# KwonGihyun/TweedieMix

Measured on AMD Instinct MI355X. Metric: denoise steps/sec @ SDXL 1024^2 K=3 concepts (fusion phase); images/sec at 1/2/4/8 GPUs, higher is better.
Workload: dtype bf16

## Files before the change

include/tmix.h:

```cpp
#ifndef TMIX_H
#define TMIX_H

#include <stdint.h>

#ifdef __cplusplus
extern "C" {
#endif

#define TMIX_VERSION 100

enum { TMIX_OK = 0, TMIX_EINVAL = -1, TMIX_ESHAPE = -2, TMIX_EARCH = -3, TMIX_EALIGN = -4 };
enum { TMIX_F32 = 0, TMIX_F16 = 1, TMIX_BF16 = 2 };

int tmix_version(void);
const char* tmix_last_error_string(void);
int tmix_check_device(void);
void tmix_env_refresh(void);

int tmix_prof_begin(uint64_t* slots, int capacity, int detail);
int tmix_prof_end(void);

enum { TMIX_STEP_FUSION = 0, TMIX_STEP_PLAIN = 1, TMIX_STEP_RESAMPLE = 2 };
int tmix_fused_tweedie_step(const float* x, const void* eps, int eps_dtype, const float* masks,
                            float* out_x, float* out_x0, int K, int channels, int64_t hw, int mode,
// ... 9 lines not shown
                                     int64_t keep_eps_seed_stride, const float* keep_w, int64_t keep_w_seed_stride, void* stream);
int tmix_fused_tweedie_step_ms_dev(const float* x, const void* eps, int eps_dtype, const float* masks,
                                   int64_t mask_seed_stride, float* out_x, float* out_x0, float* x0_prev, int K, int channels,
                                   int64_t hw, int mode, int rows, int seeds, const float* params, void* stream);
int64_t tmix_cfg_rescale_ws_doubles(int rows, int seeds);
int tmix_cfg_rescale_factors(const void* eps, int eps_dtype, float* factors, double* ws, int K, int channels, int64_t hw, int mode,
                             int rows, int seeds, const float* params, int g_slot, float phi, void* stream);
int tmix_fused_tweedie_step_rs_dev(const float* x, const void* eps, int eps_dtype, const float* masks,
                                   int64_t mask_seed_stride, float* out_x, float* out_x0, int K, int channels,
                                   int64_t hw, int mode, int rows, int seeds, const float* params, const float* factors, void* stream);
int tmix_fused_tweedie_step_ms_rs_dev(const float* x, const void* eps, int eps_dtype, const float* masks,
                                      int64_t mask_seed_stride, float* out_x, float* out_x0, float* x0_prev, int K, int channels,
                                      int64_t hw, int mode, int rows, int seeds, const float* params, const float* factors, void* stream);
int tmix_step_prologue(const float* x, float* latent, float* t_dev, const float* params, int seeds, int rows,
                       int64_t n, void* stream);
#define TMIX_MAX_WINDOWS 8
int tmix_window_consensus(float* x, int groups, int n_win, const int* win_yx, int C, int h, int w, int canvas_h, int canvas_w,
                          const float* weight, void* stream);
#define TMIX_EDT_NONE (1 << 30)
int tmix_mask_edt(const float* mask, int32_t* d_set, int32_t* d_clear, int n, int h, int w, void* stream);
int tmix_soft_masks(const int32_t* d_set, const int32_t* d_clear, float* out, int n_sets, int K, int h, int w, float feather,
                    float dilate, int normalize, void* stream);
#define TMIX_SHAPE_FILL_HOLES 1
#define TMIX_SHAPE_RESOLVE    2
#define TMIX_SHAPE_MAX_PIXELS 16384
int tmix_mask_label(const float* map, float threshold, int invert, int32_t* label, int n, int h, int w, void* stream);
int tmix_attn_shapes(const float* score, float* out, int n_sets, int km1, int h, int w, float threshold, int flags, void* stream);

int tmix_vpred_step(const void* x, const void* v, void* out, int dtype, int64_t n, float g,
                    float sa, float s1, float sa_next, float s1_next, void* stream);
// ... 76 lines not shown
    int32_t batch_bias_images;
    float* col_stats_out;
    const void* S1; const void* S2;
    int32_t S1_channels, S2_channels;
} tmix_conv_desc;
int tmix_conv3x3_nhwc(const tmix_conv_desc* d, void* stream);
int tmix_conv3x3_nhwc_fp8(const tmix_conv_desc* d, const uint8_t* scale_x, const uint8_t* scale_w, void* stream);
int tmix_conv_resolve_tile(const tmix_conv_desc* d, int fp8_operands);

int tmix_conv_in(const float* x_nchw, const float* w_ohwi, const float* bias, void* y_nhwc,
                 int B, int Cin, int H, int W, int Cout, void* stream);
int tmix_conv_in_pre(const float* x_nchw, const float* w_ohwi, const float* bias, void* y_nhwc,
                     int B, int Cin, int H, int W, int Cout, const float* pre_w, const float* pre_b, void* stream);
int tmix_conv_out(const void* x_nhwc, const void* w_ohwi, const float* bias, float* y_nchw,
                  int B, int Cin, int H, int W, int Cout, void* stream);

int tmix_attn_fwd(const void* Q, int64_t ldq, int64_t strideQ, const void* K, int64_t ldk, int64_t strideK,
                  const void* Vt, int64_t ldvt, int64_t strideVt, void* O, int64_t ldo, int64_t strideO,
                  int B, int H, int Sq, int Skv, float scale, void* stream);
int tmix_attn_fwd_f8(const void* Q, int64_t ldq, int64_t strideQ, const void* K, int64_t ldk, int64_t strideK,
                     const void* Vt, int64_t ldvt, int64_t strideVt, void* O8, int64_t ldo8, void* scales, int64_t ldScale,
                     int B, int H, int Sq, int Skv, float scale, void* stream);
int64_t tmix_attn_split_ws_bytes(int B, int H, int Sq, int Skv);
int tmix_attn_fwd_ws(const void* Q, int64_t ldq, int64_t strideQ, const void* K, int64_t ldk, int64_t strideK,
                     const void* Vt, int64_t ldvt, int64_t strideVt, void* O, int64_t ldo, int64_t strideO,
                     int B, int H, int Sq, int Skv, float scale, void* ws, int64_t ws_bytes, void* stream);
int tmix_attn_fwd_f8_ws(const void* Q, int64_t ldq, int64_t strideQ, const void* K, int64_t ldk, int64_t strideK,
                        const void* Vt, int64_t ldvt, int64_t strideVt, void* O8, int64_t ldo8, void* scales, int64_t ldScale,
                        int B, int H, int Sq, int Skv, float scale, void* ws, int64_t ws_bytes, void* stream);

// ... 56 lines not shown
```

tweediemix_amd/csrc/conv_io.hip:

```cpp
#include "common.h"

namespace {

struct PreMap { float w[16]; float b[4]; int on; };

template <int CIN>
__global__ void __launch_bounds__(256) conv_in_kernel(const float* __restrict__ x, const float* __restrict__ w,
                                                      const float* __restrict__ bias, bf16_t* __restrict__ y,
                                                      int B, int H, int W, int Cout, const PreMap pm) {
    extern __shared__ __attribute__((aligned(16))) float s_w[];
    constexpr int KK = 9 * CIN;
    const int tid = threadIdx.x, lane = tid & 63;
    const int q = __builtin_amdgcn_readfirstlane(tid >> 6);
    for (int i = tid; i < Cout * KK / 4; i += 256) ((float4*)s_w)[i] = ((const float4*)w)[i];
    __syncthreads();
    const int64_t npix = (int64_t)B * H * W;
    for (int64_t tile = blockIdx.x; tile * 64 < npix; tile += gridDim.x) {
    int64_t pix = tile * 64 + lane;
    const bool live = pix < npix;
    if (!live) pix = npix - 1;
    const int b = (int)(pix / ((int64_t)H * W)); const int rem = (int)(pix - (int64_t)b * H * W);
    const int oy = rem / W, ox = rem - oy * W;
    float patch[KK];
#pragma unroll
// ... 31 lines not shown
    }
    }
}

template <int CIN>
int launch_conv_in(unsigned nb, int smem, hipStream_t st, const float* x, const float* w, const float* bias, bf16_t* y, int B, int H, int W, int Cout, const PreMap& pm) {
    static int attr_smem = 0;
    if (smem > 64 * 1024 && smem > attr_smem) {
        hipError_t e = hipFuncSetAttribute((const void*)conv_in_kernel<CIN>, hipFuncAttributeMaxDynamicSharedMemorySize, smem);
        if (e != hipSuccess) TMIX_FAIL((int)e, "hipFuncSetAttribute: %s", hipGetErrorString(e));
        attr_smem = smem;
    }
    conv_in_kernel<CIN><<<nb, 256, smem, st>>>(x, w, bias, y, B, H, W, Cout, pm);
    TMIX_LAUNCH_CHECK();
    return TMIX_OK;
}

__global__ void __launch_bounds__(256) conv_out_kernel(const bf16_t* __restrict__ x, const bf16_t* __restrict__ w,
                                                       const float* __restrict__ bias, float* __restrict__ y,
                                                       int B, int H, int W, int Cin, int Cout) {
    const int lane = threadIdx.x & 63, fr = lane & 15, fg = lane >> 4;
    const int64_t npix = (int64_t)B * H * W;
    const int64_t pbase = ((int64_t)blockIdx.x * 4 + (threadIdx.x >> 6)) * 16;
    if (pbase >= npix) return;
    int64_t pix = pbase + fr; if (pix > npix - 1) pix = npix - 1;
    const int b = (int)(pix / ((int64_t)H * W)); const int rem = (int)(pix - (int64_t)b * H * W);
    const int oy = rem / W, ox = rem - oy * W;
    const int co = fr < Cout ? fr : Cout - 1;
    const bf16_t* wrow = w + (int64_t)co * 9 * Cin;
    f32x4 acc = {0.f, 0.f, 0.f, 0.f};
// ... 49 lines not shown
    PreMap pm = {};
    if (pre_w) {
        pm.on = 1;
        for (int i = 0; i < 16; ++i) pm.w[i] = pre_w[i];
        for (int i = 0; i < 4; ++i) pm.b[i] = pre_b ? pre_b[i] : 0.f;
    }
    hipStream_t st = (hipStream_t)stream;
    bf16_t* y = (bf16_t*)y_nhwc;
    switch (Cin) {
        case 8:  return launch_conv_in<8>(nb, smem, st, x_nchw, w_ohwi, bias, y, B, H, W, Cout, pm);
        case 3:  return launch_conv_in<3>(nb, smem, st, x_nchw, w_ohwi, bias, y, B, H, W, Cout, pm);
        default: return launch_conv_in<4>(nb, smem, st, x_nchw, w_ohwi, bias, y, B, H, W, Cout, pm);
    }
}

extern "C" int tmix_conv_out(const void* x_nhwc, const void* w_ohwi, const float* bias, float* y_nchw,
                             int B, int Cin, int H, int W, int Cout, void* stream) {
    if (!x_nhwc || !w_ohwi || !y_nchw) TMIX_FAIL(TMIX_EINVAL, "conv_out: null pointer");
    if (B <= 0 || H <= 0 || W <= 0 || Cout <= 0 || Cout > 16 || (Cin % 32)) TMIX_FAIL(TMIX_ESHAPE, "conv_out: Cin=%d (%%32) Cout=%d (<=16)", Cin, Cout);
    if (!aligned16(x_nhwc) || !aligned16(w_ohwi)) TMIX_FAIL(TMIX_EALIGN, "conv_out: pointers must be 16-byte aligned");
    const int64_t npix = (int64_t)B * H * W;
    const unsigned nb = (unsigned)((npix + 63) / 64);
    conv_out_kernel<<<nb, 256, 0, (hipStream_t)stream>>>((const bf16_t*)x_nhwc, (const bf16_t*)w_ohwi, bias, y_nchw, B, H, W, Cin, Cout);
    TMIX_LAUNCH_CHECK();
    return TMIX_OK;
}
```

tweediemix_amd/csrc/tweedie_step.hip:

```cpp
#include "common.h"

namespace {

template <int DT> struct EpsT;
template <> struct EpsT<TMIX_F32>  { typedef float  T; static __device__ __forceinline__ float ld(const float* p, int64_t i) { return p[i]; } };
template <> struct EpsT<TMIX_F16>  { typedef __half T; static __device__ __forceinline__ float ld(const __half* p, int64_t i) { return __half2float(p[i]); } };
template <> struct EpsT<TMIX_BF16> { typedef bf16_t T; static __device__ __forceinline__ float ld(const bf16_t* p, int64_t i) { return bf2f(p[i]); } };

template <int DT> __device__ __forceinline__ float rnd(float v) {
    if constexpr (DT == TMIX_F16) {
        asm volatile("" : "+v"(v));
        return __half2float(__float2half_rn(v));
    } else return v;
}

template <int DT> __device__ __forceinline__ float cfg(float eu, float ec, float g) {
    const float d = rnd<DT>(ec - eu);
    const float gd = rnd<DT>(g * d);
    return rnd<DT>(eu + gd);
}

struct KeepArgs { const float* x0; const float* eps; const float* w; int64_t x0_stride, eps_stride, w_stride; };
__device__ __forceinline__ KeepArgs keep_args(const KeepArgs& k) { return k; }
struct RescaleArgs { const float* fac; };
// ... 108 lines not shown
    int64_t bx = (n + 255) / 256; if (bx > 2048) bx = 2048;
    const dim3 grid((unsigned)bx, (unsigned)seeds);
    const T* e = (const T*)eps;
    switch (mode) {
    case TMIX_STEP_FUSION:
        tweedie_step_kernel<DT, TMIX_STEP_FUSION, 1><<<grid, 256, 0, st>>>(x, e, masks, out_x, out_x0, K, n, hw, 0.f, 1.f, 0.f, 1.f, 0.f, 0, prm, rows, mss, kp); break;
    case TMIX_STEP_PLAIN:
        tweedie_step_kernel<DT, TMIX_STEP_PLAIN, 1><<<grid, 256, 0, st>>>(x, e, masks, out_x, out_x0, K, n, hw, 0.f, 1.f, 0.f, 1.f, 0.f, 0, prm, rows, mss, kp); break;
    default:
        tweedie_step_kernel<DT, TMIX_STEP_RESAMPLE, 1><<<grid, 256, 0, st>>>(x, e, masks, out_x, out_x0, K, n, hw, 0.f, 1.f, 0.f, 1.f, 0.f, 0, prm, rows, mss, kp); break;
    }
    TMIX_LAUNCH_CHECK();
    return TMIX_OK;
}

__global__ void __launch_bounds__(256)
step_prologue_kernel(const float* __restrict__ x, float* __restrict__ latent, float* __restrict__ t_dev,
                     const float* __restrict__ prm, int rows, int64_t n) {
    const int64_t sd = blockIdx.y;
    const float4* src = (const float4*)(x + sd * n);
    for (int64_t i = (int64_t)blockIdx.x * blockDim.x + threadIdx.x; i < n / 4; i += (int64_t)gridDim.x * blockDim.x) {
        const float4 v = src[i];
        for (int r = 0; r < rows; ++r) ((float4*)(latent + (sd * rows + r) * n))[i] = v;
    }
    if (blockIdx.x == 0 && threadIdx.x < rows) t_dev[sd * rows + threadIdx.x] = prm[0];
}


template <int DT>
__global__ void __launch_bounds__(256)
vpred_step_kernel(const typename EpsT<DT>::T* __restrict__ x, const typename EpsT<DT>::T* __restrict__ v,
                  typename EpsT<DT>::T* __restrict__ out, int64_t n, float g, float sa, float s1, float sa_n, float s1_n) {
    const int64_t stride = (int64_t)gridDim.x * blockDim.x;
    for (int64_t i = (int64_t)blockIdx.x * blockDim.x + threadIdx.x; i < n; i += stride) {
        const float xv = EpsT<DT>::ld(x, i);
        const float vv = cfg<DT>(EpsT<DT>::ld(v, i), EpsT<DT>::ld(v, n + i), g);
        const float eps = rnd<DT>(rnd<DT>(sa * vv) + rnd<DT>(s1 * xv));
        const float x0 = rnd<DT>(rnd<DT>(sa * xv) - rnd<DT>(s1 * vv));
        StT<DT>::st(out, i, rnd<DT>(rnd<DT>(sa_n * x0) + rnd<DT>(s1_n * eps)));
    }
// ... 181 lines not shown
    }
    TMIX_FAIL(TMIX_EINVAL, "tweedie_step_rs_dev: bad eps dtype %d", eps_dtype);
}

extern "C" int tmix_step_prologue(const float* x, float* latent, float* t_dev, const float* params, int seeds, int rows,
                                  int64_t n, void* stream) {
    if (!x || !latent || !t_dev || !params) TMIX_FAIL(TMIX_EINVAL, "step_prologue: null pointer");
    if (seeds < 1 || seeds > 65535 || rows < 1 || rows > 256 || n < 4 || (n & 3)) TMIX_FAIL(TMIX_ESHAPE, "step_prologue: seeds=%d rows=%d n=%lld (n %% 4 == 0)", seeds, rows, (long long)n);
    if (!aligned16(x) || !aligned16(latent)) TMIX_FAIL(TMIX_EALIGN, "step_prologue: x / latent must be 16-byte aligned");
    int64_t bx = (n / 4 + 255) / 256; if (bx > 256) bx = 256;
    step_prologue_kernel<<<dim3((unsigned)bx, (unsigned)seeds), 256, 0, (hipStream_t)stream>>>(x, latent, t_dev, params, rows, n);
    TMIX_LAUNCH_CHECK();
    return TMIX_OK;
}

extern "C" int tmix_video_step_prologue(const float* x, float* x_u, int64_t clip_stride_u, float* t_u, float* x_c, int64_t clip_stride_c,
                                        float* t_c, const float* params, int videos, int channels, int frames, int64_t hw,
                                        int row_channels, void* stream) {
    if (!x || !x_u || !t_u || !x_c || !t_c || !params) TMIX_FAIL(TMIX_EINVAL, "video_step_prologue: null pointer");
    if (videos < 1 || channels < 1 || frames < 1 || hw < 1 || row_channels < channels)
        TMIX_FAIL(TMIX_ESHAPE, "video_step_prologue: videos=%d channels=%d frames=%d hw=%lld row_channels=%d", videos, channels, frames, (long long)hw, row_channels);
    const int64_t clip = (int64_t)frames * row_channels * hw;
    if (clip_stride_u < clip || clip_stride_c < clip)
        TMIX_FAIL(TMIX_ESHAPE, "video_step_prologue: clip strides %lld / %lld < one clip's %lld floats", (long long)clip_stride_u, (long long)clip_stride_c, (long long)clip);
    const int64_t n = (int64_t)videos * channels * frames * hw;
    int64_t blocks = (n + 255) / 256; if (blocks > 4096) blocks = 4096;
    video_prologue_kernel<<<(unsigned)blocks, 256, 0, (hipStream_t)stream>>>(x, x_u, clip_stride_u, t_u, x_c, clip_stride_c, t_c, params,
                                                                             videos, channels, frames, hw, row_channels, n);
    TMIX_LAUNCH_CHECK();
    return TMIX_OK;
// ... 18 lines not shown
```

tweediemix_amd/lib.py:

```python
from __future__ import annotations

import ctypes as C
import os

_HERE = os.path.dirname(os.path.abspath(__file__))
LIB_PATH = os.path.join(_HERE, "lib", "libtmix_hip.so")
LIB_PATH = os.environ.get("TMIX_LIB", LIB_PATH)

OK, EINVAL, ESHAPE, EARCH, EALIGN = 0, -1, -2, -3, -4
F32, F16, BF16 = 0, 1, 2
STEP_FUSION, STEP_PLAIN, STEP_RESAMPLE = 0, 1, 2
EPI_NONE, EPI_GEGLU, EPI_F32OUT, EPI_GELU, EPI_QUICKGELU = 0, 1, 2, 3, 4
CONV_S1, CONV_S2, CONV_UP2, CONV_T3, CONV_S2A, CONV_UP2F = 0, 1, 2, 3, 4, 5
F8_A_BLOCK_SCALES, F8_GEGLU_OUT, F8_COPY_OUT = 1, 2, 4
MAX_WINDOWS = 8
EDT_NONE = 1 << 30
SHAPE_FILL_HOLES, SHAPE_RESOLVE, SHAPE_MAX_PIXELS = 1, 2, 16384
TILE_AUTO, TILE_COUNT = 0, 26
TILE_CANDIDATES = (1, 2, 3, 4, 5, 7, 12, 13, 14, 15, 16, 17, 18, 19, 20, 21, 22)
TILE_EXCLUSIVE = (13, 14, 15, 22, 24)
TILE_CONV_HALO = 26

i32, i64, f32, vp = C.c_int32, C.c_int64, C.c_float, C.c_void_p

# ... 32 lines not shown
    "tmix_fused_tweedie_step": (C.c_int, [vp, vp, C.c_int, vp, vp, vp, C.c_int, C.c_int, i64, C.c_int,
                                          f32, f32, f32, f32, f32, C.c_int, vp]),
    "tmix_fused_tweedie_step_dev": (C.c_int, [vp, vp, C.c_int, vp, i64, vp, vp, C.c_int, C.c_int, i64, C.c_int, C.c_int,
                                              C.c_int, vp, vp]),
    "tmix_fused_tweedie_step_keep_dev": (C.c_int, [vp, vp, C.c_int, vp, i64, vp, vp, C.c_int, C.c_int, i64, C.c_int, C.c_int,
                                                   C.c_int, vp, vp, i64, vp, i64, vp, i64, vp]),
    "tmix_fused_tweedie_step_ms_dev": (C.c_int, [vp, vp, C.c_int, vp, i64, vp, vp, vp, C.c_int, C.c_int, i64, C.c_int, C.c_int,
                                                 C.c_int, vp, vp]),
    "tmix_cfg_rescale_ws_doubles": (i64, [C.c_int, C.c_int]),
    "tmix_cfg_rescale_factors": (C.c_int, [vp, C.c_int, vp, vp, C.c_int, C.c_int, i64, C.c_int, C.c_int, C.c_int, vp, C.c_int, f32, vp]),
    "tmix_fused_tweedie_step_rs_dev": (C.c_int, [vp, vp, C.c_int, vp, i64, vp, vp, C.c_int, C.c_int, i64, C.c_int, C.c_int,
                                                 C.c_int, vp, vp, vp]),
    "tmix_fused_tweedie_step_ms_rs_dev": (C.c_int, [vp, vp, C.c_int, vp, i64, vp, vp, vp, C.c_int, C.c_int, i64, C.c_int, C.c_int,
                                                    C.c_int, vp, vp, vp]),
    "tmix_step_prologue": (C.c_int, [vp, vp, vp, vp, C.c_int, C.c_int, i64, vp]),
    "tmix_window_consensus": (C.c_int, [vp, C.c_int, C.c_int, C.POINTER(C.c_int32), C.c_int, C.c_int, C.c_int, C.c_int, C.c_int, vp, vp]),
    "tmix_mask_edt": (C.c_int, [vp, vp, vp, C.c_int, C.c_int, C.c_int, vp]),
    "tmix_soft_masks": (C.c_int, [vp, vp, vp, C.c_int, C.c_int, C.c_int, C.c_int, f32, f32, C.c_int, vp]),
    "tmix_mask_label": (C.c_int, [vp, f32, C.c_int, vp, C.c_int, C.c_int, C.c_int, vp]),
    "tmix_attn_shapes": (C.c_int, [vp, vp, C.c_int, C.c_int, C.c_int, C.c_int, f32, C.c_int, vp]),
    "tmix_gemm_bf16": (C.c_int, [C.POINTER(GemmDesc), vp]),
    "tmix_gemm_prefetch_next": (C.c_int, [vp, i64, vp]),
    "tmix_gemm_fp8": (C.c_int, [C.POINTER(GemmDesc), vp, vp, vp]),
    "tmix_gemm_q_cross_attn": (C.c_int, [C.POINTER(GemmDesc), vp, i64, i64, vp, i64, i64, vp, i64, C.c_int, C.c_int, f32, vp]),
    "tmix_quantize_fp8_rows": (C.c_int, [vp, i64, vp, i64, vp, i64, C.c_int, vp]),
    "tmix_conv3x3_nhwc": (C.c_int, [C.POINTER(ConvDesc), vp]),
    "tmix_conv3x3_nhwc_fp8": (C.c_int, [C.POINTER(ConvDesc), vp, vp, vp]),
    "tmix_conv_in": (C.c_int, [vp, vp, vp, vp, C.c_int, C.c_int, C.c_int, C.c_int, C.c_int, vp]),
    "tmix_conv_in_pre": (C.c_int, [vp, vp, vp, vp, C.c_int, C.c_int, C.c_int, C.c_int, C.c_int, vp, vp, vp]),
    "tmix_softmax_rows": (C.c_int, [vp, i64, vp, i64, i64, C.c_int, f32, vp]),
    "tmix_softmax_rows_causal": (C.c_int, [vp, i64, vp, i64, i64, C.c_int, f32, C.c_int, vp]),
    "tmix_softmax_rows_masked": (C.c_int, [vp, i64, vp, i64, i64, C.c_int, C.c_int, f32, vp]),
    "tmix_affine_clamp": (C.c_int, [vp, vp, i64, f32, f32, f32, f32, vp]),
    "tmix_conv_out": (C.c_int, [vp, vp, vp, vp, C.c_int, C.c_int, C.c_int, C.c_int, C.c_int, vp]),
    "tmix_attn_fwd": (C.c_int, [vp, i64, i64, vp, i64, i64, vp, i64, i64, vp, i64, i64,
                                C.c_int, C.c_int, C.c_int, C.c_int, f32, vp]),
    "tmix_attn_fwd_f8": (C.c_int, [vp, i64, i64, vp, i64, i64, vp, i64, i64, vp, i64, vp, i64,
                                   C.c_int, C.c_int, C.c_int, C.c_int, f32, vp]),
    "tmix_attn_split_ws_bytes": (i64, [C.c_int, C.c_int, C.c_int, C.c_int]),
    "tmix_attn_fwd_ws": (C.c_int, [vp, i64, i64, vp, i64, i64, vp, i64, i64, vp, i64, i64,
                                   C.c_int, C.c_int, C.c_int, C.c_int, f32, vp, i64, vp]),
    "tmix_attn_fwd_f8_ws": (C.c_int, [vp, i64, i64, vp, i64, i64, vp, i64, i64, vp, i64, vp, i64,
                                      C.c_int, C.c_int, C.c_int, C.c_int, f32, vp, i64, vp]),
    "tmix_groupnorm_nhwc_launches": (C.c_int, [i64, C.c_int, C.c_int]),
    "tmix_groupnorm_ws_chunks": (C.c_int, [i64]),
    "tmix_groupnorm_ws_floats": (i64, [C.c_int, C.c_int, C.c_int]),
    "tmix_groupnorm_nhwc": (C.c_int, [vp, C.c_int, vp, C.c_int, vp, vp, vp, vp, C.c_int, i64, C.c_int, f32,
                                      C.c_int, vp]),
    "tmix_groupnorm_nhwc_pre": (C.c_int, [vp, C.c_int, vp, C.c_int, vp, vp, vp, vp, C.c_int, i64, C.c_int, f32,
# ... 65 lines not shown
```

tweediemix_amd/ops.py:

```python
from __future__ import annotations

import ctypes as C
import os

import numpy as np
import torch

from . import lib as L

BF16 = torch.bfloat16


def _stream() -> int:
    return torch.cuda.current_stream().cuda_stream


def _p(t):
    return None if t is None else t.data_ptr()


def _need_cuda(*ts):
    for t in ts:
        if t is not None and not t.is_cuda:
            raise L.TmixError("tweediemix_amd ops need device tensors (no CPU fallback exists)")
# ... 477 lines not shown
    return out


def conv_in(x_nchw, w_ohwi, bias, out=None):
    _need_cuda(x_nchw, w_ohwi)
    lib = L.load()
    B, Cin, H, W = x_nchw.shape
    Cout = w_ohwi.shape[0]
    assert x_nchw.dtype == torch.float32 and w_ohwi.dtype == torch.float32 and x_nchw.is_contiguous() and w_ohwi.is_contiguous()
    if out is None:
        out = torch.empty(B, H, W, Cout, device=x_nchw.device, dtype=BF16)
    L.check(lib.tmix_conv_in(_p(x_nchw), _p(w_ohwi), _p(bias), _p(out), B, Cin, H, W, Cout, _stream()), "tmix_conv_in")
    return out


def conv_out(x_nhwc, w_ohwi, bias, out=None):
    _need_cuda(x_nhwc, w_ohwi)
    lib = L.load()
    B, H, W, Cin = x_nhwc.shape
    Cout = w_ohwi.shape[0]
    assert x_nhwc.dtype == BF16 and w_ohwi.dtype == BF16 and x_nhwc.is_contiguous() and w_ohwi.is_contiguous()
    if out is None:
        out = torch.empty(B, Cout, H, W, device=x_nhwc.device, dtype=torch.float32)
    L.check(lib.tmix_conv_out(_p(x_nhwc), _p(w_ohwi), _p(bias), _p(out), B, Cin, H, W, Cout, _stream()), "tmix_conv_out")
    return out


def attention_split_ws(B, H, Sq, Skv, device):
    n = L.load().tmix_attn_split_ws_bytes(B, H, Sq, Skv)
    return torch.zeros(n, device=device, dtype=torch.uint8) if n > 0 else None


def attention(q, k, vt, H, Skv, scale, out=None, f8_out=None, ws=None):
    _need_cuda(q, k, vt)
    lib = L.load()
    B, Sq = q.shape[0], q.shape[1]
    assert q.dtype == BF16 and k.dtype == BF16 and vt.dtype == BF16
    assert q.stride(2) == 1 and k.stride(2) == 1 and vt.stride(2) == 1
    wsa = (ws.data_ptr(), ws.numel()) if ws is not None else (None, 0)
# ... 348 lines not shown
```

tweediemix_amd/sampler.py:

```python
from __future__ import annotations

from types import SimpleNamespace

import torch

from . import lib as L
from . import ops
from .schedule import Schedule
from .guidance import validate_phi
from .solver import SOLVERS, multistep_coeffs
from .unet import KVCache, PlanGroup, TokenMapSpec, TokenPropSpec, UNetPlan, UNetWeights

F32 = torch.float32


def seed_everything(seed: int):
    import random

    import numpy as np
    torch.manual_seed(seed)
    if torch.cuda.is_available():
        torch.cuda.manual_seed(seed)
    random.seed(seed)
    np.random.seed(seed)
# ... 75 lines not shown
                                 + (f"; unknown keys {sorted(extra)}" if extra else ""))
            self.mask_soften = dict(feather=f, dilate=r, normalize=bool(ms.get("normalize", False)))
        self._mask_buf = None
        self.scheduler = Schedule(config.n_timesteps, spacing=timestep_spacing)
        self.skip = self.scheduler.skip
        self.final_alpha_cumprod = self.scheduler.final_alpha_cumprod
        self.h, self.w = config.resolution_h // 8, config.resolution_w // 8
        self.canvas_h, self.canvas_w = self.h, self.w
        if canvas is not None:
            self._init_canvas(dict(canvas), attention_masks)
        self.add_time_ids = torch.tensor([[config.resolution_h, config.resolution_w, config.crops_coords_top_left_h,
                                           config.crops_coords_top_left_w, config.resolution_h, config.resolution_w]],
                                         dtype=F32)
        self.plans = {}
        self.graphs = {}
        self.unet_calls = []
        self.preview_x0 = None
        S = self.n_seeds
        self.x_state = torch.zeros(S, 4, self.h, self.w, device=self.device, dtype=F32)
        self.x0_state = torch.zeros_like(self.x_state)
        self._x_backup = torch.zeros_like(self.x_state)
        self._x_look = torch.zeros_like(self.x_state) if (self.attention_masks or {}).get("propagate") else None
        self.step_params = torch.zeros(8, device=self.device, dtype=F32)
        self._x0_prev = torch.zeros_like(self.x_state) if solver != "ddim" else None
        self._ms_last = None
        self._rs_rows = max(self.concept_num + 1, 2)
        self._rs_factors = self._rs_ws = None
        if self.guidance_rescale > 0.0:
            self._rs_factors = torch.ones(S * (self._rs_rows - 1), device=self.device, dtype=F32)
            self._rs_ws = ops.cfg_rescale_ws(self._rs_rows, S, self.device)
# ... 111 lines not shown
                            fp8=self.fp8, token_maps=spec)
        if kind == "propagate":
            am = self.attention_masks
            spec = TokenPropSpec(len(am["flat"]), row0=1, row_step=2, n_rows=S, levels=am["levels"])
            return UNetPlan(self.W, B, self.h, self.w, KVCache(self.W, ehs, wsel), pooled, self.add_time_ids.repeat(B, 1),
                            fp8=self.fp8, token_prop=spec)
        if self.n_streams > 1 and B % self.n_streams == 0 and B // self.n_streams >= self.min_rows_per_stream:
            return PlanGroup(self.W, self.h, self.w, ehs, wsel, pooled, self.add_time_ids.repeat(B, 1), routed,
                             self.n_streams, fp8=self.fp8)
        kv = KVCache(self.W, ehs, wsel)
        return UNetPlan(self.W, B, self.h, self.w, kv, pooled, self.add_time_ids.repeat(B, 1), routed=routed,
                        row_sets=wsel if routed else None, fp8=self.fp8)

    def plan(self, kind):
        if kind not in self.plans:
            self.plans[kind] = self._build_plan(kind)
        return self.plans[kind]

    def _unet(self, kind, x, t):
        p = self.plan(kind)
        S = self.n_seeds
        self.unet_calls.append((kind, p.B // S, int(t)))
        p.latent.view(S, p.B // S, *p.latent.shape[1:]).copy_(x.unsqueeze(1))
        p.t_dev.fill_(float(t))
        p.run()
        return p.eps

    def _set_masks(self, masks):
        masks = masks.to(self.device, F32).contiguous()
        assert masks.dim() in (4, 5) and tuple(masks.shape[-4:]) == (self.concept_num, 1, self.h, self.w), tuple(masks.shape)
        if self._mask_buf is None or self._mask_buf.shape != masks.shape:
# ... 15 lines not shown

    @masks.setter
    def masks(self, m):
        if m is None:
            self._mask_buf = None
        else:
            self._set_masks(m)

    def _enqueue_step(self, kind, mode, ms=False):
        p = self.plan(kind)
        S = self.n_seeds
        rows = p.B // S
        n = 4 * self.h * self.w
        lib = L.load()
        st = torch.cuda.current_stream().cuda_stream
        L.check(lib.tmix_step_prologue(self.x_state.data_ptr(), p.latent.data_ptr(), p.t_dev.data_ptr(),
                                       self.step_params.data_ptr(), S, rows, n, st), "tmix_step_prologue")
        p.run()
        self._fused_step(p.eps.data_ptr(), L.F32, rows, mode, st, ms)
        if self.windows is not None:
            self._consensus(self.x_state)

    def _fused_step(self, eps_ptr, eps_dt, rows, mode, st, ms=False):
        lib = L.load()
        m = self._mask_buf if mode == L.STEP_FUSION else None
        mss = 0 if (m is None or m.dim() == 4) else self.concept_num * self.h * self.w
        hw = self.h * self.w
        head = (self.x_state.data_ptr(), eps_ptr, eps_dt, None if m is None else m.data_ptr(), mss, self.x_state.data_ptr(),
                self.x0_state.data_ptr(), self.concept_num, 4, hw, mode, rows, self.n_seeds, self.step_params.data_ptr())
        if self.guidance_rescale > 0.0:
            if rows > self._rs_rows:
                raise ValueError(f"guidance_rescale: {rows} eps rows per seed, the buffers were sized for {self._rs_rows}")
            L.check(lib.tmix_cfg_rescale_factors(eps_ptr, eps_dt, self._rs_factors.data_ptr(), self._rs_ws.data_ptr(), self.concept_num, 4, hw, mode,
# ... 6 lines not shown
                L.check(lib.tmix_fused_tweedie_step_rs_dev(*head, self._rs_factors.data_ptr(), st), "tmix_fused_tweedie_step_rs_dev")
            return
        if ms:
            L.check(lib.tmix_fused_tweedie_step_ms_dev(*head[:7], self._x0_prev.data_ptr(), *head[7:], st), "tmix_fused_tweedie_step_ms_dev")
            return
        if self._keep is None:
            L.check(lib.tmix_fused_tweedie_step_dev(*head, st), "tmix_fused_tweedie_step_dev")
            return
        kx, kw, ke = self._keep
        L.check(lib.tmix_fused_tweedie_step_keep_dev(*head, kx.data_ptr(), 0 if kx.shape[0] == 1 else 4 * hw, ke.data_ptr(), 4 * hw,
                                                     kw.data_ptr(), 0 if kw.shape[0] == 1 else hw, st), "tmix_fused_tweedie_step_keep_dev")

    def _run_step(self, kind, mode, t, at, at_next, is_last=False, ms=None):
        if "_unet" not in vars(self):
            self.unet_calls.append((kind, self.plan(kind).B // self.n_seeds, int(t)))
        sa, s1, san, s1n = ops.step_coeffs(at, at_next)
        i = self._hp_i
        self._hp_i = (i + 1) % self._hp.shape[0]
        if self._hp_ev[i] is not None:
            self._hp_ev[i].synchronize()
        hp = self._hp[i]
        if ms is None:
            hp[0], hp[1], hp[2], hp[3], hp[4] = float(t), sa, s1, san, s1n
            hp[5], hp[6] = (1.0 if is_last else 0.0), float(self.config.guidance_scale)
        else:
            hp[0], hp[1], hp[2], hp[3], hp[4], hp[5] = float(t), sa, s1, ms[0], ms[1], ms[2]
            hp[6], hp[7] = (1.0 if is_last else 0.0), float(self.config.guidance_scale)
        self.step_params.copy_(hp, non_blocking=True)
        if self.device.type == "cuda":
            self._hp_ev[i] = torch.cuda.Event()
# ... 1 lines not shown
        if mode == L.STEP_FUSION:
            assert self._mask_buf is not None, "fusion step before the masks were acquired"
        if "_unet" in vars(self):
            eps = self._unet(kind, self.x_state, t).contiguous()
            self._fused_step(eps.data_ptr(), ops._EPS_DT[eps.dtype], eps.shape[0] // self.n_seeds, mode,
                             torch.cuda.current_stream().cuda_stream, ms is not None)
            if self.windows is not None:
                self._consensus(self.x_state)
            return
        if not self.use_graphs:
            self._enqueue_step(kind, mode, ms is not None)
            return
        gkey = (kind, mode, "ms") if ms is not None else (kind, mode) if self._keep is None else (kind, mode, "keep")
        if self.guidance_rescale > 0.0:
            gkey = gkey + ("rs",)
        g = self.graphs.get(gkey)
        if g is None:
            self._enqueue_step(kind, mode, ms is not None)
            torch.cuda.synchronize()
            g = torch.cuda.CUDAGraph()
            keep = self.x_state.clone()
            with torch.cuda.graph(g):
                self._enqueue_step(kind, mode, ms is not None)
            self.x_state.copy_(keep)
            self.graphs[gkey] = g
            return
        g.replay()

    def _decode(self, latent, inv_scale):
        if self.vae is None:
# ... 200 lines not shown
```

tweediemix_amd/unet.py:

```python
from __future__ import annotations

import ctypes as C
import json
import os
from dataclasses import dataclass

import torch

from . import lib as L
from . import ops
from .plan import LaunchPlan, hint_bytes
from .weights import LOG2E, fold_layernorm, interleave_geglu, q_log2_units

BF16 = torch.bfloat16
F32 = torch.float32


@dataclass
class UNetConfig:
    in_channels: int = 4
    out_channels: int = 4
    block_out_channels: tuple = (320, 640, 1280)
    layers_per_block: int = 2
    transformer_layers: tuple = (0, 2, 10)
# ... 842 lines not shown
        thid = torch.empty(B, T, device=self.dev, dtype=F32)
        emb = torch.empty(B, T, device=self.dev, dtype=F32)
        self.keep += [tsin, thid, emb]
        self._emit(lib.tmix_timestep_embedding, self.t_dev.data_ptr(), tsin.data_ptr(), B, C0)
        self._emit(lib.tmix_linear_small, tsin.data_ptr(), W["time_embedding.linear_1.weight"].data_ptr(),
                   W["time_embedding.linear_1.bias"].data_ptr(), None, thid.data_ptr(), B, T, C0, 0, 1)
        self._emit(lib.tmix_linear_small, thid.data_ptr(), W["time_embedding.linear_2.weight"].data_ptr(),
                   W["time_embedding.linear_2.bias"].data_ptr(), self.aug.data_ptr(), emb.data_ptr(), B, T, T, 0, 1)
        tw, tb_, starts, names = W.stacked_time_proj()
        tall = torch.empty(B * tw.shape[0], device=self.dev, dtype=F32)
        self.keep.append(tall)
        self._emit(lib.tmix_linear_small_sections, emb.data_ptr(), tw.data_ptr(), tb_.data_ptr(), tall.data_ptr(), B, tw.shape[0], T, 0,
                   starts.data_ptr(), len(names))
        hs = starts.tolist()
        self._temb = {n: tall[hs[i] * B:hs[i + 1] * B].view(B, hs[i + 1] - hs[i]) for i, n in enumerate(names)}
        Hh, Ww = self.h, self.w
        x = A.get(B, Hh * Ww, C0)
        self._emit(lib.tmix_conv_in, self.latent.data_ptr(), W["conv_in.weight"].data_ptr(), W["conv_in.bias"].data_ptr(),
                   x.data_ptr(), B, cfg.in_channels, Hh, Ww, C0)
        skips = [(x, C0)]
        ci = C0
        for bi, co in enumerate(ch):
            for j in range(cfg.layers_per_block):
                xin = x
                x = self._resnet(xin, ci, co, Hh, Ww, f"down_blocks.{bi}.resnets.{j}", emb)
                if cfg.transformer_layers[bi]:
                    x2 = self._t2d(x, co, Hh, Ww, f"down_blocks.{bi}.attentions.{j}", cfg.transformer_layers[bi])
                    A.put(x)
                    x = x2
                ci = co
# ... 32 lines not shown
                x = x2
                Hh, Ww = Hh * 2, Ww * 2
        y = self._gn(x, C0, Hh * Ww, "conv_norm_out", 1e-5, True)
        A.put(x)
        self._emit(lib.tmix_conv_out, y.data_ptr(), W["conv_out.weight"].data_ptr(), W["conv_out.bias"].data_ptr(),
                   self.eps.data_ptr(), B, C0, Hh, Ww, cfg.out_channels)
        self.flops += 2 * B * Hh * Ww * 9 * (cfg.in_channels * C0 + C0 * cfg.out_channels)
        self._freeze()

    def __call__(self, latent, t):
        self.latent.copy_(latent)
        self.t_dev.fill_(float(t))
        self.run()
        return self.eps

    def norm_condition(self, latent, t):
        self.latent.copy_(latent)
        self.t_dev.fill_(float(t))
        st = torch.cuda.current_stream().cuda_stream
        prods = {id(d) for d, _c in self._ln_links}
        out = []
        for i, (fn, args) in enumerate(self.ops):
            rc = fn(*args, st)
            if rc:
                L.check(rc, fn.__name__)
            m = self.op_meta.get(i)
            if not m or m[0] not in ("gemm", "gemm_fp8") or id(m[2]) not in prods:
                continue
            d = m[2]
            torch.cuda.synchronize()
# ... 168 lines not shown
```

Baseline: 32.62.

## Precompute timestep embedding table and add tiled LDS conv_out kernel

Precomputes the per-timestep time-embedding projections for every scheduler timestep once at plan build. The step prologue then copies the matching table row into the projection buffer, skipping the timestep embedding and linear ops each step. Separately, conv_out gets a tiled kernel that stages a halo tile of the NHWC input in shared memory and runs MFMA 16x16x32 bf16 over the 9 taps, falling back to the old direct kernel when shared memory would be too large. The cost is extra device memory for the table and a NaN-filled fallback path when a timestep is missing from the table.

```diff
diff --git a/include/tmix.h b/include/tmix.h
--- a/include/tmix.h
+++ b/include/tmix.h
@@ -47,6 +47,8 @@
                                       int64_t hw, int mode, int rows, int seeds, const float* params, const float* factors, void* stream);
 int tmix_step_prologue(const float* x, float* latent, float* t_dev, const float* params, int seeds, int rows,
                        int64_t n, void* stream);
+int tmix_step_prologue_table(const float* x, float* latent, float* t_dev, const float* params, int seeds, int rows, int64_t n,
+                             const float* table, const float* ts, int n_t, int64_t row_floats, float* tall, void* stream);
 #define TMIX_MAX_WINDOWS 8
 int tmix_window_consensus(float* x, int groups, int n_win, const int* win_yx, int C, int h, int w, int canvas_h, int canvas_w,
                           const float* weight, void* stream);
@@ -153,6 +155,8 @@
                      int B, int Cin, int H, int W, int Cout, const float* pre_w, const float* pre_b, void* stream);
 int tmix_conv_out(const void* x_nhwc, const void* w_ohwi, const float* bias, float* y_nchw,
                   int B, int Cin, int H, int W, int Cout, void* stream);
+int tmix_conv_out_direct(const void* x_nhwc, const void* w_ohwi, const float* bias, float* y_nchw,
+                         int B, int Cin, int H, int W, int Cout, void* stream);
 
 int tmix_attn_fwd(const void* Q, int64_t ldq, int64_t strideQ, const void* K, int64_t ldk, int64_t strideK,
                   const void* Vt, int64_t ldvt, int64_t strideVt, void* O, int64_t ldo, int64_t strideO,
diff --git a/tweediemix_amd/csrc/conv_io.hip b/tweediemix_amd/csrc/conv_io.hip
--- a/tweediemix_amd/csrc/conv_io.hip
+++ b/tweediemix_amd/csrc/conv_io.hip
@@ -69,6 +69,90 @@
     conv_in_kernel<CIN><<<nb, 256, smem, st>>>(x, w, bias, y, B, H, W, Cout, pm);
     TMIX_LAUNCH_CHECK();
     return TMIX_OK;
+}
+
+constexpr int CO_TH = 4, CO_TW = 16, CO_HW = CO_TW + 2, CO_HPIX = (CO_TH + 2) * CO_HW;
+static inline int conv_out_tile_smem(int Cin) { return CO_HPIX * (Cin * 2 + 16); }
+
+template <int CO_STAGE>
+__global__ void __launch_bounds__(256) conv_out_tile_kernel(const bf16_t* __restrict__ x, const bf16_t* __restrict__ w,
+                                                            const float* __restrict__ bias, float* __restrict__ y,
+                                                            int B, int H, int W, int Cin, int Cout, int tiles_x, int tiles_y, int vec4) {
+    extern __shared__ __attribute__((aligned(16))) unsigned char s_x[];
+    const int tid = threadIdx.x, lane = tid & 63, fr = lane & 15, fg = lane >> 4;
+    const int wv = __builtin_amdgcn_readfirstlane(tid >> 6);
+    int t = xcd_remap(blockIdx.x, gridDim.x);
+    const int tx = t % tiles_x; t /= tiles_x;
+    const int ty = t % tiles_y, b = t / tiles_y;
+    const int y0 = ty * CO_TH, x0 = tx * CO_TW;
+    const int cpp = Cin >> 3, pitch = Cin * 2 + 16;
+    const int total = CO_HPIX * cpp;
+    const bf16_t* xb = x + (int64_t)b * H * W * Cin;
+    const int co = fr < Cout ? fr : Cout - 1;
+    const bf16_t* wp = w + (int64_t)co * 9 * Cin + fg * 8;
+    frag_ab ra[3], rw[9];
+#pragma unroll
+    for (int j = 0; j < 9; ++j) rw[j] = *(const frag_ab*)(wp + 32 * j);
+    {
+        int hp = tid / cpp, ch = tid - hp * cpp;
+        const int dp = 256 / cpp, dc = 256 - dp * cpp;
+        for (int i0 = tid; i0 < total; i0 += 256 * CO_STAGE) {
+            uint4 v[CO_STAGE]; int off[CO_STAGE]; bool in[CO_STAGE];
+#pragma unroll
+            for (int j = 0; j < CO_STAGE; ++j) {
+                const bool past = i0 + j * 256 >= total;
+                const int hq = past ? CO_HPIX - 1 : hp, cq = past ? cpp - 1 : ch;
+                const int hy = hq / CO_HW, hx = hq - hy * CO_HW;
+                const int iy = y0 + hy - 1, ix = x0 + hx - 1;
+                in[j] = iy >= 0 && iy < H && ix >= 0 && ix < W;
+                const int cy = iy < 0 ? 0 : (iy > H - 1 ? H - 1 : iy), cx = ix < 0 ? 0 : (ix > W - 1 ? W - 1 : ix);
+                v[j] = *(const uint4*)(xb + ((int64_t)cy * W + cx) * Cin + cq * 8);
+                off[j] = hq * pitch + cq * 16;
+                hp += dp; ch += dc;
+                if (ch >= cpp) { ch -= cpp; ++hp; }
+            }
+#pragma unroll
+            for (int j = 0; j < CO_STAGE; ++j) *(uint4*)(s_x + off[j]) = in[j] ? v[j] : make_uint4(0, 0, 0, 0);
+        }
+    }
+    __syncthreads();
+    const int oy = y0 + wv;
+    if (oy >= H) return;
+    const int ks = Cin >> 5, nsteps = 9 * ks;
+    const unsigned char* abase = s_x + (wv * CO_HW + fr) * pitch + fg * 16;
+    int ptap = 0, pcc = 0;
+    auto fetch_a = [&](frag_ab& a) {
+        const int tp = ptap < 9 ? ptap : 0;
+        const int ky = tp / 3, kx = tp - ky * 3;
+        a = *(const frag_ab*)(abase + (ky * CO_HW + kx) * pitch + pcc * 64);
+        if (++pcc == ks) { pcc = 0; ++ptap; }
+    };
+#pragma unroll
+    for (int j = 0; j < 3; ++j) fetch_a(ra[j]);
+#pragma unroll
+    for (int j = 0; j < 9; ++j) asm volatile("" : "+v"(rw[j]));
+    f32x4 acc = {0.f, 0.f, 0.f, 0.f};
+    for (int s = 0; s < nsteps; s += 9) {
+        const bool more = s + 9 < nsteps;
+#pragma unroll
+        for (int j = 0; j < 9; ++j) {
+            acc = __builtin_amdgcn_mfma_f32_16x16x32_bf16(ra[j % 3], rw[j], acc, 0, 0, 0);
+            fetch_a(ra[j % 3]);
+            rw[j] = *(const frag_ab*)(wp + 32 * (more ? s + 9 + j : j));
+            __builtin_amdgcn_sched_barrier(0);
+        }
+    }
+    if (fr < Cout) {
+        const float bv = bias ? bias[fr] : 0.f;
+        const int ox = x0 + fg * 4;
+        float* dst = y + (((int64_t)b * Cout + fr) * H + oy) * W + ox;
+        if (vec4 && ox < W) *(float4*)dst = make_float4(acc[0] + bv, acc[1] + bv, acc[2] + bv, acc[3] + bv);
+        else {
+#pragma unroll
+            for (int r = 0; r < 4; ++r)
+                if (ox + r < W) dst[r] = acc[r] + bv;
+        }
+    }
 }
 
 __global__ void __launch_bounds__(256) conv_out_kernel(const bf16_t* __restrict__ x, const bf16_t* __restrict__ w,
@@ -148,14 +232,42 @@
     }
 }
 
-extern "C" int tmix_conv_out(const void* x_nhwc, const void* w_ohwi, const float* bias, float* y_nchw,
-                             int B, int Cin, int H, int W, int Cout, void* stream) {
+static int conv_out_check(const void* x_nhwc, const void* w_ohwi, const float* y_nchw, int B, int Cin, int H, int W, int Cout) {
     if (!x_nhwc || !w_ohwi || !y_nchw) TMIX_FAIL(TMIX_EINVAL, "conv_out: null pointer");
-    if (B <= 0 || H <= 0 || W <= 0 || Cout <= 0 || Cout > 16 || (Cin % 32)) TMIX_FAIL(TMIX_ESHAPE, "conv_out: Cin=%d (%%32) Cout=%d (<=16)", Cin, Cout);
+    if (B <= 0 || H <= 0 || W <= 0 || Cin <= 0 || Cout <= 0 || Cout > 16 || (Cin % 32)) TMIX_FAIL(TMIX_ESHAPE, "conv_out: Cin=%d (%%32) Cout=%d (<=16)", Cin, Cout);
     if (!aligned16(x_nhwc) || !aligned16(w_ohwi)) TMIX_FAIL(TMIX_EALIGN, "conv_out: pointers must be 16-byte aligned");
+    return TMIX_OK;
+}
+
+extern "C" int tmix_conv_out_direct(const void* x_nhwc, const void* w_ohwi, const float* bias, float* y_nchw,
+                                    int B, int Cin, int H, int W, int Cout, void* stream) {
+    if (int rc = conv_out_check(x_nhwc, w_ohwi, y_nchw, B, Cin, H, W, Cout)) return rc;
     const int64_t npix = (int64_t)B * H * W;
     const unsigned nb = (unsigned)((npix + 63) / 64);
     conv_out_kernel<<<nb, 256, 0, (hipStream_t)stream>>>((const bf16_t*)x_nhwc, (const bf16_t*)w_ohwi, bias, y_nchw, B, H, W, Cin, Cout);
     TMIX_LAUNCH_CHECK();
     return TMIX_OK;
 }
+
+extern "C" int tmix_conv_out(const void* x_nhwc, const void* w_ohwi, const float* bias, float* y_nchw,
+                             int B, int Cin, int H, int W, int Cout, void* stream) {
+    if (int rc = conv_out_check(x_nhwc, w_ohwi, y_nchw, B, Cin, H, W, Cout)) return rc;
+    const int smem = conv_out_tile_smem(Cin);
+    const int64_t tiles_x = (W + CO_TW - 1) / CO_TW, tiles_y = (H + CO_TH - 1) / CO_TH, nb = (int64_t)B * tiles_y * tiles_x;
+    if (smem > 160 * 1024 || nb > 0x7fffffff)
+        return tmix_conv_out_direct(x_nhwc, w_ohwi, bias, y_nchw, B, Cin, H, W, Cout, stream);
+    const int vec4 = (W % 4 == 0) && aligned16(y_nchw);
+    const bf16_t* x = (const bf16_t*)x_nhwc; const bf16_t* w = (const bf16_t*)w_ohwi;
+    if (CO_HPIX * (Cin / 8) > 9 * 256) {
+        static int attr_smem = 0;
+        if (smem > 64 * 1024 && smem > attr_smem) {
+            hipError_t e = hipFuncSetAttribute((const void*)conv_out_tile_kernel<18>, hipFuncAttributeMaxDynamicSharedMemorySize, smem);
+            if (e != hipSuccess) TMIX_FAIL((int)e, "hipFuncSetAttribute: %s", hipGetErrorString(e));
+            attr_smem = smem;
+        }
+        conv_out_tile_kernel<18><<<(unsigned)nb, 256, smem, (hipStream_t)stream>>>(x, w, bias, y_nchw, B, H, W, Cin, Cout, (int)tiles_x, (int)tiles_y, vec4);
+    } else
+        conv_out_tile_kernel<9><<<(unsigned)nb, 256, smem, (hipStream_t)stream>>>(x, w, bias, y_nchw, B, H, W, Cin, Cout, (int)tiles_x, (int)tiles_y, vec4);
+    TMIX_LAUNCH_CHECK();
+    return TMIX_OK;
+}
diff --git a/tweediemix_amd/csrc/tweedie_step.hip b/tweediemix_amd/csrc/tweedie_step.hip
--- a/tweediemix_amd/csrc/tweedie_step.hip
+++ b/tweediemix_amd/csrc/tweedie_step.hip
@@ -146,9 +146,8 @@
     return TMIX_OK;
 }
 
-__global__ void __launch_bounds__(256)
-step_prologue_kernel(const float* __restrict__ x, float* __restrict__ latent, float* __restrict__ t_dev,
-                     const float* __restrict__ prm, int rows, int64_t n) {
+__device__ __forceinline__ void prologue_rows(const float* __restrict__ x, float* __restrict__ latent, float* __restrict__ t_dev,
+                                              const float* __restrict__ prm, int rows, int64_t n) {
     const int64_t sd = blockIdx.y;
     const float4* src = (const float4*)(x + sd * n);
     for (int64_t i = (int64_t)blockIdx.x * blockDim.x + threadIdx.x; i < n / 4; i += (int64_t)gridDim.x * blockDim.x) {
@@ -156,6 +155,37 @@
         for (int r = 0; r < rows; ++r) ((float4*)(latent + (sd * rows + r) * n))[i] = v;
     }
     if (blockIdx.x == 0 && threadIdx.x < rows) t_dev[sd * rows + threadIdx.x] = prm[0];
+}
+
+__global__ void __launch_bounds__(256)
+step_prologue_kernel(const float* __restrict__ x, float* __restrict__ latent, float* __restrict__ t_dev,
+                     const float* __restrict__ prm, int rows, int64_t n) {
+    prologue_rows(x, latent, t_dev, prm, rows, n);
+}
+
+__global__ void __launch_bounds__(256)
+step_prologue_table_kernel(const float* __restrict__ x, float* __restrict__ latent, float* __restrict__ t_dev,
+                           const float* __restrict__ prm, int rows, int64_t n, const float* __restrict__ table,
+                           const float* __restrict__ ts, int n_t, int64_t row_floats, float* __restrict__ tall) {
+    prologue_rows(x, latent, t_dev, prm, rows, n);
+    if (blockIdx.y != 0) return;
+    __shared__ int s_idx;
+    if (threadIdx.x == 0) s_idx = -1;
+    __syncthreads();
+    const float t = prm[0];
+    for (int i = threadIdx.x; i < n_t; i += blockDim.x)
+        if (ts[i] == t) s_idx = i;
+    __syncthreads();
+    const int idx = s_idx;
+    float4* dst = (float4*)tall;
+    const int64_t n4 = row_floats / 4, stride = (int64_t)gridDim.x * blockDim.x;
+    if (idx >= 0) {
+        const float4* row = (const float4*)(table + (int64_t)idx * row_floats);
+        for (int64_t i = (int64_t)blockIdx.x * blockDim.x + threadIdx.x; i < n4; i += stride) dst[i] = row[i];
+    } else {
+        const float q = __uint_as_float(0x7fc00000u);
+        for (int64_t i = (int64_t)blockIdx.x * blockDim.x + threadIdx.x; i < n4; i += stride) dst[i] = make_float4(q, q, q, q);
+    }
 }
 
 
@@ -367,6 +397,18 @@
     return TMIX_OK;
 }
 
+extern "C" int tmix_step_prologue_table(const float* x, float* latent, float* t_dev, const float* params, int seeds, int rows, int64_t n,
+                                        const float* table, const float* ts, int n_t, int64_t row_floats, float* tall, void* stream) {
+    if (!x || !latent || !t_dev || !params || !table || !ts || !tall) TMIX_FAIL(TMIX_EINVAL, "step_prologue_table: null pointer");
+    if (seeds < 1 || seeds > 65535 || rows < 1 || rows > 256 || n < 4 || (n & 3)) TMIX_FAIL(TMIX_ESHAPE, "step_prologue_table: seeds=%d rows=%d n=%lld (n %% 4 == 0)", seeds, rows, (long long)n);
+    if (n_t < 1 || n_t > 65536 || row_floats < 4 || (row_floats & 3)) TMIX_FAIL(TMIX_ESHAPE, "step_prologue_table: n_t=%d row_floats=%lld (%% 4 == 0)", n_t, (long long)row_floats);
+    if (!aligned16(x) || !aligned16(latent) || !aligned16(table) || !aligned16(tall)) TMIX_FAIL(TMIX_EALIGN, "step_prologue_table: x / latent / table / tall must be 16-byte aligned");
+    int64_t bx = (n / 4 + 255) / 256; if (bx > 256) bx = 256;
+    step_prologue_table_kernel<<<dim3((unsigned)bx, (unsigned)seeds), 256, 0, (hipStream_t)stream>>>(x, latent, t_dev, params, rows, n, table, ts, n_t, row_floats, tall);
+    TMIX_LAUNCH_CHECK();
+    return TMIX_OK;
+}
+
 extern "C" int tmix_video_step_prologue(const float* x, float* x_u, int64_t clip_stride_u, float* t_u, float* x_c, int64_t clip_stride_c,
                                         float* t_c, const float* params, int videos, int channels, int frames, int64_t hw,
                                         int row_channels, void* stream) {
diff --git a/tweediemix_amd/lib.py b/tweediemix_amd/lib.py
--- a/tweediemix_amd/lib.py
+++ b/tweediemix_amd/lib.py
@@ -70,6 +70,7 @@
     "tmix_fused_tweedie_step_ms_rs_dev": (C.c_int, [vp, vp, C.c_int, vp, i64, vp, vp, vp, C.c_int, C.c_int, i64, C.c_int, C.c_int,
                                                     C.c_int, vp, vp, vp]),
     "tmix_step_prologue": (C.c_int, [vp, vp, vp, vp, C.c_int, C.c_int, i64, vp]),
+    "tmix_step_prologue_table": (C.c_int, [vp, vp, vp, vp, C.c_int, C.c_int, i64, vp, vp, C.c_int, i64, vp, vp]),
     "tmix_window_consensus": (C.c_int, [vp, C.c_int, C.c_int, C.POINTER(C.c_int32), C.c_int, C.c_int, C.c_int, C.c_int, C.c_int, vp, vp]),
     "tmix_mask_edt": (C.c_int, [vp, vp, vp, C.c_int, C.c_int, C.c_int, vp]),
     "tmix_soft_masks": (C.c_int, [vp, vp, vp, C.c_int, C.c_int, C.c_int, C.c_int, f32, f32, C.c_int, vp]),
@@ -89,6 +90,7 @@
     "tmix_softmax_rows_masked": (C.c_int, [vp, i64, vp, i64, i64, C.c_int, C.c_int, f32, vp]),
     "tmix_affine_clamp": (C.c_int, [vp, vp, i64, f32, f32, f32, f32, vp]),
     "tmix_conv_out": (C.c_int, [vp, vp, vp, vp, C.c_int, C.c_int, C.c_int, C.c_int, C.c_int, vp]),
+    "tmix_conv_out_direct": (C.c_int, [vp, vp, vp, vp, C.c_int, C.c_int, C.c_int, C.c_int, C.c_int, vp]),
     "tmix_attn_fwd": (C.c_int, [vp, i64, i64, vp, i64, i64, vp, i64, i64, vp, i64, i64,
                                 C.c_int, C.c_int, C.c_int, C.c_int, f32, vp]),
     "tmix_attn_fwd_f8": (C.c_int, [vp, i64, i64, vp, i64, i64, vp, i64, i64, vp, i64, vp, i64,
diff --git a/tweediemix_amd/ops.py b/tweediemix_amd/ops.py
--- a/tweediemix_amd/ops.py
+++ b/tweediemix_amd/ops.py
@@ -515,7 +515,7 @@
     return out
 
 
-def conv_out(x_nhwc, w_ohwi, bias, out=None):
+def conv_out(x_nhwc, w_ohwi, bias, out=None, direct=False):
     _need_cuda(x_nhwc, w_ohwi)
     lib = L.load()
     B, H, W, Cin = x_nhwc.shape
@@ -523,7 +523,8 @@
     assert x_nhwc.dtype == BF16 and w_ohwi.dtype == BF16 and x_nhwc.is_contiguous() and w_ohwi.is_contiguous()
     if out is None:
         out = torch.empty(B, Cout, H, W, device=x_nhwc.device, dtype=torch.float32)
-    L.check(lib.tmix_conv_out(_p(x_nhwc), _p(w_ohwi), _p(bias), _p(out), B, Cin, H, W, Cout, _stream()), "tmix_conv_out")
+    fn = lib.tmix_conv_out_direct if direct else lib.tmix_conv_out
+    L.check(fn(_p(x_nhwc), _p(w_ohwi), _p(bias), _p(out), B, Cin, H, W, Cout, _stream()), "tmix_conv_out")
     return out
 
 
diff --git a/tweediemix_amd/sampler.py b/tweediemix_amd/sampler.py
--- a/tweediemix_amd/sampler.py
+++ b/tweediemix_amd/sampler.py
@@ -113,6 +113,7 @@
                                          dtype=F32)
         self.plans = {}
         self.graphs = {}
+        self._time_hit = True
         self.unet_calls = []
         self.preview_x0 = None
         S = self.n_seeds
@@ -254,7 +255,9 @@
 
     def plan(self, kind):
         if kind not in self.plans:
-            self.plans[kind] = self._build_plan(kind)
+            p = self.plans[kind] = self._build_plan(kind)
+            if isinstance(p, UNetPlan) and kind not in ("probe", "propagate"):
+                p.build_time_table(self.scheduler.timesteps)
         return self.plans[kind]
 
     def _unet(self, kind, x, t):
@@ -300,9 +303,15 @@
         n = 4 * self.h * self.w
         lib = L.load()
         st = torch.cuda.current_stream().cuda_stream
-        L.check(lib.tmix_step_prologue(self.x_state.data_ptr(), p.latent.data_ptr(), p.t_dev.data_ptr(),
-                                       self.step_params.data_ptr(), S, rows, n, st), "tmix_step_prologue")
-        p.run()
+        if getattr(p, "time_table", None) is not None and self._time_hit:
+            L.check(lib.tmix_step_prologue_table(self.x_state.data_ptr(), p.latent.data_ptr(), p.t_dev.data_ptr(), self.step_params.data_ptr(), S, rows, n,
+                                                 p.time_table.data_ptr(), p.time_ts.data_ptr(), p.time_table.shape[0], p.time_table.shape[1],
+                                                 p._tall.data_ptr(), st), "tmix_step_prologue_table")
+            p.run_after_time()
+        else:
+            L.check(lib.tmix_step_prologue(self.x_state.data_ptr(), p.latent.data_ptr(), p.t_dev.data_ptr(),
+                                           self.step_params.data_ptr(), S, rows, n, st), "tmix_step_prologue")
+            p.run()
         self._fused_step(p.eps.data_ptr(), L.F32, rows, mode, st, ms)
         if self.windows is not None:
             self._consensus(self.x_state)
@@ -339,6 +348,7 @@
     def _run_step(self, kind, mode, t, at, at_next, is_last=False, ms=None):
         if "_unet" not in vars(self):
             self.unet_calls.append((kind, self.plan(kind).B // self.n_seeds, int(t)))
+            self._time_hit = float(t) in (getattr(self.plan(kind), "time_index", None) or ())
         sa, s1, san, s1n = ops.step_coeffs(at, at_next)
         i = self._hp_i
         self._hp_i = (i + 1) % self._hp.shape[0]
@@ -370,6 +380,8 @@
         gkey = (kind, mode, "ms") if ms is not None else (kind, mode) if self._keep is None else (kind, mode, "keep")
         if self.guidance_rescale > 0.0:
             gkey = gkey + ("rs",)
+        if not self._time_hit and getattr(self.plan(kind), "time_table", None) is not None:
+            gkey = gkey + ("tc",)
         g = self.graphs.get(gkey)
         if g is None:
             self._enqueue_step(kind, mode, ms is not None)
diff --git a/tweediemix_amd/unet.py b/tweediemix_amd/unet.py
--- a/tweediemix_amd/unet.py
+++ b/tweediemix_amd/unet.py
@@ -880,6 +880,7 @@
                    starts.data_ptr(), len(names))
         hs = starts.tolist()
         self._temb = {n: tall[hs[i] * B:hs[i + 1] * B].view(B, hs[i + 1] - hs[i]) for i, n in enumerate(names)}
+        self._tall, self._n_time_ops = tall, len(self.ops)
         Hh, Ww = self.h, self.w
         x = A.get(B, Hh * Ww, C0)
         self._emit(lib.tmix_conv_in, self.latent.data_ptr(), W["conv_in.weight"].data_ptr(), W["conv_in.bias"].data_ptr(),
@@ -942,6 +943,33 @@
         self.run()
         return self.eps
 
+    time_table = time_ts = time_index = None
+
+    def build_time_table(self, timesteps, max_bytes=128 << 20):
+        ts = [float(t) for t in timesteps]
+        n = self._tall.numel()
+        if os.environ.get("TMIX_TIME_TABLE", "1") == "0" or not ts or len(set(ts)) != len(ts) or n % 4 or len(ts) * n * 4 > max_bytes:
+            return False
+        table = torch.empty(len(ts), n, device=self.dev, dtype=F32)
+        st = torch.cuda.current_stream().cuda_stream
+        for i, t in enumerate(ts):
+            self.t_dev.fill_(t)
+            for fn, args in self.ops[:self._n_time_ops]:
+                L.check(fn(*args, st), fn.__name__)
+            table[i].copy_(self._tall)
+        self.time_table, self.time_ts = table, torch.tensor(ts, device=self.dev, dtype=F32)
+        self.time_index = {t: i for i, t in enumerate(ts)}
+        return True
+
+    def run_after_time(self, stream=None):
+        st = stream if stream is not None else torch.cuda.current_stream().cuda_stream
+        ops_ = self.ops
+        for i in range(self._n_time_ops, len(ops_)):
+            fn, args = ops_[i]
+            rc = fn(*args, st)
+            if rc:
+                L.check(rc, fn.__name__)
+
     def norm_condition(self, latent, t):
         self.latent.copy_(latent)
         self.t_dev.fill_(float(t))
```

New measurement: 32.72 (median of 6 runs). No clear change (+0.3%).
